# yinwoods/k8s-scheduler

Hardware: AMD Instinct MI355X
Metric: pod-node evaluations/sec (higher is better)
Workload: dtype f64

## Files before the change

### k8s-scheduler_amd/csrc/ksched_commit.h

```cpp
#pragma once

#include <hip/hip_runtime.h>

#include <type_traits>

#ifndef KSCHED_XCHG_DEBUG
#define KSCHED_XCHG_DEBUG 0
#endif

#include "ksched_pipe.h"

namespace ksched {

namespace {

constexpr int kSpcHashBits = 11;
constexpr int kSpcHash = 1 << kSpcHashBits;
template <bool LAG3>
constexpr int spc_slots() { return LAG3 ? 192 : 128; }
static_assert(spc_slots<true>() + 1 <= kRescueMaxT, "RescueReq::ti must hold the persistent commit's touched slots");
constexpr int kSpcInvalid = kSpcHash - 1;
constexpr int kGS = 14;

constexpr uint64_t kSkipKeyBits = 0x7ff8000000000badull;
__device__ __forceinline__ double skip_key() { return __longlong_as_double((long long)kSkipKeyBits); }
__device__ __forceinline__ float screen_y(int64_t a, double y) {
    return (a > 0 && a < (1ll << 52)) ? (float)y : __builtin_nanf("");
}

struct alignas(16) TouchY {
    float c, m, p, w;
};
__device__ __forceinline__ TouchY touch_stage(int64_t a0, int64_t a1, int64_t a2, double y0, double y1, double y2) {
    return TouchY{screen_y(a0, y0), screen_y(a1, y1), screen_y(a2, y2), 0.0f};
}
__device__ __forceinline__ bool touch_need(float qc, float qm, float qp, float thr, const TouchY &ty, int64_t rc, int64_t rm,
                                           int64_t rp, int64_t n0, int64_t n1, int64_t n2, bool active, float *v) {
    bool lo;
    *v = screen_pair(qc, qm, qp, ty.c, ty.m, ty.p, n0 >= rc, n1 >= rm, n2 >= rp, &lo);
    return active && !(*v < thr);
// ... 47 lines not shown
    int32_t *gs;
    double *pbk;
    int64_t *pbx;
    int32_t *ctl;
    int32_t *own;
    uint64_t *GS;
    float *thr;
    int16_t *x2s;
    float *rb2;
};

__device__ __forceinline__ uint32_t spc_hash(int32_t idx) {
    return ((uint32_t)idx * 2654435761u) >> (32 - kSpcHashBits);
}

__device__ __forceinline__ int spc_pos_insert(int32_t *hk, int32_t idx, bool *existed = nullptr) {
    uint32_t h = spc_hash(idx);
    for (;;) {
        if (h != kSpcInvalid) {
            const int32_t prev = atomicCAS(&hk[h], -1, idx);
            if (prev == -1 || prev == idx) {
                if (existed) *existed = prev == idx;
                return (int)h;
            }
        }
        h = (h + 1) & (kSpcHash - 1);
    }
}

__device__ __forceinline__ int64_t rl64(int64_t v, int src) {
    const uint32_t hi = (uint32_t)__builtin_amdgcn_readlane((int)((uint64_t)v >> 32), src);
    const uint32_t lo = (uint32_t)__builtin_amdgcn_readlane((int)(uint32_t)(uint64_t)v, src);
    return (int64_t)(((uint64_t)hi << 32) | lo);
}

__device__ __forceinline__ void persist_plan(const CommitArgs &A, bool truncated, int64_t cursor) {
    PersistLocal *L = A.loc;
    const int64_t n1 = L->plan[(A.batch + kPipeLag - 1) % kPlanRing];
    int64_t nx = truncated ? cursor : (n1 < 0 ? -1 : n1 + A.B);
    if (nx >= A.pods.p) nx = -1;
    L->plan[(A.batch + kPipeLag) % kPlanRing] = nx;
    st_coh(A.plan2, (uint64_t)nx);
}

__device__ __forceinline__ void stage_state(double *o, const int64_t *a) {
    for (int r = 0; r < 3; ++r) {
        const double f = (double)a[r];
        o[r] = f;
        o[3 + r] = recip_or_zero(a[r], f);
    }
}

__device__ __forceinline__ void lds_order() {
    __builtin_amdgcn_fence(__ATOMIC_RELEASE, "wavefront");
    __builtin_amdgcn_wave_barrier();
    __builtin_amdgcn_fence(__ATOMIC_ACQUIRE, "wavefront");
}

template <int PRIO, int DOM, bool LAB, bool F53>
__device__ __forceinline__ double lane_key(bool f, int64_t rc, int64_t rm, int64_t rp, double rcf, double rmf,
                                           double rpf, int64_t n0, int64_t n1, int64_t n2, double y3, float pr) {
    const double nf0 = (double)n0, nf1 = (double)n1, nf2 = (double)n2;
    const double ny0 = recip_or_zero(n0, nf0), ny1 = recip_or_zero(n1, nf1), ny2 = recip_or_zero(n2, nf2);
    double k;
    const bool el = pair_key_fast<PRIO, DOM, F53>(f, rc, rm, rp, rcf, rmf, rpf, n0, n1, n2, nf0, nf1, nf2, ny0, ny1,
                                                  ny2, y3, pr, &k);
// ... 180 lines not shown
            if (wave == 0) {
                if (lane == 0) {
                    L->cursor = ho.cursor;
                    L->plan[(A.batch + kPipeLag - 1) % kPlanRing] = ho.plan_next;
                    L->rseq = ho.rseq;
                    persist_plan(A, false, ho.cursor);
                    st_coh(A.cursor_at, (uint64_t)ho.cursor);
                    drain_stores();
                    put_handoff(A.ctl, A.batch, 0, ho.cursor, ho.rseq, L->plan[(A.batch + kPipeLag) % kPlanRing]);
                }
                publish_committed<COH>(A);
            }
            return 1;
        }
    } else {
        const int64_t cursor = load_i64<COH>(&A.ctl->cursor);
        if (p0 < 0 || p0 >= A.pods.p || p0 != cursor) {
            if (!wait()) return 0;
            if (wave == 0) {
                if (lane == 0) {
                    A.xout->count = 0;
                    if (p0 >= 0 && p0 < A.pods.p) add_i64<COH>(&A.ctl->stats[3], 1);
                    plan_after_commit<COH>(A, false, cursor);
                }
                publish_committed<COH>(A);
            }
            return 1;
        }
    }
    const bool dbg = A.dbg != nullptr;
    uint64_t t_start = dbg ? __builtin_amdgcn_s_memtime() : 0;
    uint64_t t_pre = 0;
    uint64_t t_s1 = 0, t_s2 = 0, t_s3 = 0, t_mark = 0;
    SpcSmem m;
    {
        char *p = smem;
        m.pbk = reinterpret_cast<double *>(p); p += (size_t)kSpcWaves * 64 * sizeof(double);
        m.pbx = reinterpret_cast<int64_t *>(p); p += (size_t)kSpcWaves * 64 * sizeof(int64_t);
        m.LK = reinterpret_cast<double *>(p); p += (size_t)K * 64 * sizeof(double);
        m.GS = reinterpret_cast<uint64_t *>(p); p += 64 * kGS * sizeof(uint64_t);
        m.D = reinterpret_cast<int8_t *>(p); p += 64 * 64;
        m.T = reinterpret_cast<SpcSlot *>(p); p += (size_t)spc_slots<LAG3>() * sizeof(SpcSlot);
        m.LI = reinterpret_cast<int32_t *>(p); p += (size_t)K * 64 * sizeof(int32_t);
        m.HP = reinterpret_cast<int32_t *>(p); p += (size_t)K * 64 * sizeof(int32_t);
        m.hk = reinterpret_cast<int32_t *>(p); p += kSpcHash * sizeof(int32_t);
        m.tkc = reinterpret_cast<uint32_t *>(p); p += 64 * sizeof(uint32_t);
        m.ti = reinterpret_cast<int32_t *>(p); p += spc_slots<LAG3>() * sizeof(int32_t);
        m.fcg = reinterpret_cast<int32_t *>(p); p += 64 * sizeof(int32_t);
        m.dfacc = reinterpret_cast<int32_t *>(p); p += 64 * sizeof(int32_t);
        m.gn = reinterpret_cast<int32_t *>(p); p += 64 * sizeof(int32_t);
        m.gq = reinterpret_cast<int32_t *>(p); p += 64 * sizeof(int32_t);
        m.gs = reinterpret_cast<int32_t *>(p); p += 64 * sizeof(int32_t);
        m.ctl = reinterpret_cast<int32_t *>(p); p += 4 * sizeof(int32_t);
        m.thr = reinterpret_cast<float *>(p); p += 64 * sizeof(float);
        m.x2s = reinterpret_cast<int16_t *>(p); p += 64 * sizeof(int16_t);
        m.S = reinterpret_cast<double *>(p);
        m.own = reinterpret_cast<int32_t *>(m.pbk);
        m.s0 = reinterpret_cast<int64_t *>(m.D);
        m.iy = reinterpret_cast<double *>(m.GS);
        m.iyt = reinterpret_cast<TouchY *>(m.iy + 128 * 6);
        m.rb2 = reinterpret_cast<float *>(m.dfacc);
    }
    const int nb = (int)((A.pods.p - p0 < A.B) ? A.pods.p - p0 : A.B);
    const bool pj = lane < nb;
    const LanePods lp = pre ? *pre : load_lane_pods<LAB>(A.pods, p0, nb);
    const int64_t rc = lp.rc, rm = lp.rm, rp = lp.rp;
// ... 204 lines not shown
            L->rseq = ho.rseq;
        }
        if (p0 != ho.cursor) {
            if (wave == 0) {
                if (lane == 0) {
                    __hip_atomic_fetch_add(reinterpret_cast<unsigned long long *>(&A.ctl->stats[3]), 1ull,
                                           __ATOMIC_RELAXED, __HIP_MEMORY_SCOPE_AGENT);
                    persist_plan(A, false, ho.cursor);
                    st_coh(A.cursor_at, (uint64_t)ho.cursor);
                    drain_stores();
                    put_handoff(A.ctl, A.batch, 0, ho.cursor, ho.rseq, L->plan[(A.batch + kPipeLag) % kPlanRing]);
                }
                publish_committed<COH>(A);
            }
            return 1;
        }
        n1 = ho.n1;
#if KSCHED_XCHG_DEBUG
        if (A.xp && A.xp->xdbg && wave == 0) {
            int64_t x = lane < n1 ? (int64_t)dbg_mix((uint64_t)xi.idx ^ ((uint64_t)xi.cur[0] << 20), (uint64_t)xi.cur[1] ^
                                                     (uint64_t)xi.cur[2] ^ (uint64_t)xi.sb[0], lane) : 0;
            x = wave_sum_i64(x);
            dbg_x1 = (uint64_t)x;
        }
#endif
        if (wave == 0) {
            int h = 0;
            bool dup = false;
            if (lane < n1) {
                h = spc_pos_insert(m.hk, xi.idx);
                dup = (m.tkc[h >> 5] >> (h & 31)) & 1u;
            }
            const uint64_t nm = __ballot(lane < n1 && !dup);
            const int slot = dup ? m.own[h] : n2 + __popcll(nm & ((1ull << lane) - 1ull));
            if (lane < n1) {
                SpcSlot &x = m.T[slot];
                x.idx = xi.idx; x.mine = 0;
                for (int r = 0; r < 3; ++r) { m.s0[lane * 3 + r] = xi.sb[r]; x.sb[r] = xi.cur[r]; x.cur[r] = xi.cur[r]; }
                x.labels = xi.labels; x.price = xi.price; x.pad = 0;
                m.ti[slot] = xi.idx;
                m.gs[lane] = slot;
                if constexpr (SCR) {
                    double st[6];
                    stage_state(st, xi.cur);
#pragma unroll
                    for (int r = 0; r < 6; ++r) m.iy[lane * 6 + r] = st[r];
                    m.iyt[lane] = touch_stage(xi.cur[0], xi.cur[1], xi.cur[2], st[3], st[4], st[5]);
                } else {
                    stage_state(m.iy + lane * 6, xi.cur);
                }
                if (dup) m.x2s[slot] = -1;
                else atomicOr(&m.tkc[h >> 5], 1u << (h & 31));
            }
            if (lane == 0) m.ctl[3] = n2 + __popcll(nm);
        }
        __syncthreads();
        if (tid == 0 && A.trace_row) A.trace_row[23] = wall_clock64();
        nin = m.ctl[3];
        key_inherited(n1, [&](int e) { return (int)m.gs[e]; });
        __syncthreads();
        if (tid == 0 && A.trace_row) A.trace_row[24] = wall_clock64();
    }

    int32_t fcc = 0;
    double rbk = -__builtin_inf();
    int32_t rbi = kNoIdx, rbs = -1;
    constexpr bool RB2 = COH && PRIO == kPrioResource && DOM == kDomAll;
    bool trk = false;
    int cv = 0, cut = 0;
    int32_t my_idx = 0, my_feas = 0;
    int32_t my_src = 0;
    double my_score = 0.0;
    int32_t my_g = -2, my_q = -1, my_s = -1, my_h = kSpcInvalid;
    int nT = nin, done = nb, W = 64;
    int nresc = 0;
    int rcredit = 0, rmax = 0;
    if constexpr (COH) {
        const int c = A.loc->rescue_credit + A.rescue_rate;
        rcredit = c < 4 * A.rescue_cap ? c : 4 * A.rescue_cap;
        rmax = rcredit >= 2 * A.rescue_cap ? A.rescue_max : A.rescue_low;
    }
    int64_t placed = 0, nrounds = 0, nfail = 0, niters = 0, nseq = 0;
    if (wave == 0) {
        int64_t ds2 = 0;
        double xk = -__builtin_inf();
        int32_t xix = kNoIdx, xe = -1;
        if (LAG3 && A.batch >= 2 && n2 > 0 && pj) {
            ds2 = (int64_t)smv[0];
            xk = __longlong_as_double((long long)smv[1]);
            xix = (int32_t)(uint32_t)smv[2];
            xe = (int32_t)(smv[2] >> 32);
        }
        fcc = pj ? (int32_t)(fc0v + m.dfacc[lane] + ds2) : 0;
        cut = cut0;
#pragma unroll
        for (int q = 0; q < K; ++q) cv += m.LI[q * 64 + lane] != kNoIdx;
        for (int w = 0; w < kSpcWaves; ++w) {
            const double k = m.pbk[w * 64 + lane];
            const int64_t x = m.pbx[w * 64 + lane];
            const int32_t xi = (int32_t)(uint32_t)x;
            if (k != -__builtin_inf() && better(k, xi, rbk, rbi)) { rbk = k; rbi = xi; rbs = (int32_t)(x >> 32); }
        }
        if (LAG3 && xix != kNoIdx) {
            if (m.x2s[xe] >= 0) {
                if (better(xk, xix, rbk, rbi)) { rbk = xk; rbi = xix; rbs = m.x2s[xe]; }
            } else {
                for (int e = 0; e < n2; ++e) {
                    if (m.x2s[e] < 0) continue;
                    const double k = Srow[m.x2s[e]];
                    const int32_t xi = m.ti[m.x2s[e]];
                    if (k != -__builtin_inf() && better(k, xi, rbk, rbi)) { rbk = k; rbi = xi; rbs = m.x2s[e]; }
                }
            }
        }
        if (lane == 0) { m.ctl[0] = 0; m.ctl[2] = 0; }
// ... 46 lines not shown
            }
        }
        for (; t < nT; ++t) {
            const double v = Srow[t];
            const int32_t x = m.ti[t];
            const bool u0 = v != -__builtin_inf() && better(v, x, k0, i0);
            if constexpr (T2) { const double o0 = u0 ? k0 : v; q0 = o0 > q0 ? o0 : q0; }
            if (u0) { k0 = v; i0 = x; s0 = t; }
        }
        q0 = q1 > q0 ? q1 : q0;
        if (k1 != -__builtin_inf() && better(k1, i1, k0, i0)) {
            q0 = k0 > q0 ? k0 : q0;
            k0 = k1; i0 = i1; s0 = s1;
        } else {
            q0 = k1 > q0 ? k1 : q0;
        }
        rbk = k0; rbi = i0; rbs = s0;
        if constexpr (T2) m.rb2[lane] = __double2float_ru(q0);
    };
    int c = 0;
    if (COH && tid == 0 && A.trace_row) A.trace_row[25] = wall_clock64();
    uint64_t *const tr1 = (COH && tid == 0) ? A.trace_row : nullptr;
    bool first = true;
    const uint64_t t_pro = dbg ? __builtin_amdgcn_s_memtime() - t_start : 0;
    for (;;) {
        if (dbg) t_mark = __builtin_amdgcn_s_memtime();
        if (wave == 0) {
            const int cend = (c + W < nb) ? c + W : nb;
            lds_order();
            for (int w = lane * 4; w < kSpcHash; w += 256) *reinterpret_cast<int4 *>(m.own + w) = make_int4(64, 64, 64, 64);
            lds_order();
            const uint64_t fitm = __ballot(fcc != 0);
            const bool act = lane >= c && lane < cend && ((fitm >> lane) & 1);
            int32_t hp[K];
            uint32_t am = 0;
#pragma unroll
            for (int qq = 0; qq < K; ++qq) hp[qq] = m.HP[qq * 64 + lane];
#pragma unroll
            for (int qq = 0; qq < K; ++qq) {
                const int pos = hp[qq];
                am |= ((m.tkc[pos >> 5] >> (pos & 31)) & 1u) ? 0u : (1u << qq);
            }
            if (!act) am = 0;
            int32_t pq = -1, ph = kSpcInvalid;
            for (int it = 0;; ++it) {
                ++niters;
                int32_t nq = -1, nh = kSpcInvalid;
                if (am) {
#pragma unroll
                    for (int qq = K - 1; qq >= 0; --qq) {
                        const bool ok = (((am >> qq) & 1u) != 0u) & (m.own[hp[qq]] >= lane);
                        nq = ok ? qq : nq;
                        nh = ok ? hp[qq] : nh;
                    }
                }
                const bool changed = __ballot(act && nq != pq) != 0;
                if (act && pq >= 0) m.own[ph] = 64;
                lds_order();
                pq = nq; ph = nh;
                if (!changed && it > 0) break;
                if (act && pq >= 0) atomicMin(&m.own[ph], lane);
                lds_order();
            }
            const uint64_t gm = __ballot(act && pq >= 0);
            if (lane >= c && lane < cend) {
                my_g = act ? (pq >= 0 ? 0 : -1) : -2;
                my_q = pq;
                my_h = act && pq >= 0 ? ph : kSpcInvalid;
                my_s = act && pq >= 0 ? nT + __popcll(gm & ((1ull << lane) - 1ull)) : -1;
            }
            const bool in = lane >= c && lane < cend;
            if (in && my_g == 0) my_g = m.LI[my_q * 64 + lane];
            m.gn[lane] = in ? my_g : -2;
            m.gq[lane] = my_q;
            m.gs[lane] = my_s;
            m.fcg[lane] = 0;
            if (lane == 0) { m.ctl[0] = c; m.ctl[1] = cend; }
        }
        __syncthreads();
        if (first && tr1) tr1[49] = wall_clock64();
        if (dbg) { const uint64_t t = __builtin_amdgcn_s_memtime(); t_s1 += t - t_mark; t_mark = t; }
        const int rc0 = m.ctl[0], rce = m.ctl[1];
        {
            double pk = -__builtin_inf();
            int32_t pi = kNoIdx, ps = -1;
            if (wave == 0 && lane >= rc0 && lane < rce && m.gn[lane] >= 0) {
                const uint64_t *src = reinterpret_cast<const uint64_t *>(A.lists + (size_t)lane * K + m.gq[lane]) + 2;
                uint64_t v[5];
#pragma unroll
                for (int w = 0; w < 5; ++w) v[w] = COH ? ld_coh(src + w) : src[w];
                const int64_t n0 = wsub((int64_t)v[0], rc), n1 = wsub((int64_t)v[1], rm), n2 = wsub((int64_t)v[2], 1);
                const double nf0 = (double)n0, nf1 = (double)n1, nf2 = (double)n2;
                uint64_t *o = m.GS + (size_t)lane * kGS;
                if constexpr (SCR) {
                    const double ny0 = recip_or_zero(n0, nf0), ny1 = recip_or_zero(n1, nf1), ny2 = recip_or_zero(n2, nf2);
                    SpcSlot &x = m.T[my_s];
                    x.idx = my_g; x.mine = 1;
                    x.sb[0] = (int64_t)v[0]; x.sb[1] = (int64_t)v[1]; x.sb[2] = (int64_t)v[2];
                    x.cur[0] = n0; x.cur[1] = n1; x.cur[2] = n2;
                    x.labels = v[3]; x.price = __uint_as_float((uint32_t)v[4]); x.pad = 0;
                    m.ti[my_s] = my_g;
                    *reinterpret_cast<TouchY *>(o) = touch_stage(n0, n1, n2, ny0, ny1, ny2);
// ... 115 lines not shown
            if (fcj == 0) {
                kind = 0;
            } else if (my_g >= 0) {
                uk = m.LK[my_q * 64 + lane];
                kind = (has_t && better(tk, ti, uk, my_g)) ? 2 : 1;
            } else if (my_g == -2) {
                kind = 4;
            } else if (!cut) {
                kind = has_t ? 2 : 0;
            } else if (cv > 0) {
                const double lk = m.LK[(cv - 1) * 64 + lane];
                const int32_t lx = m.LI[(cv - 1) * 64 + lane];
                kind = (has_t && better(tk, ti, lk, lx)) ? 2 : 3;
            } else {
                kind = 3;
            }
            const bool guessed_commit = my_g >= 0;
            const bool valid = (kind == 0 && !guessed_commit) || (kind == 1);
            const bool inw = lane >= c && lane < cend;
            const uint64_t bad = __ballot(inw && !valid);
            int f = bad ? (int)__builtin_ctzll(bad) : cend;
            const bool conf = lane >= c && lane < f;
            if (conf) {
                my_idx = kind == 1 ? my_g : (fcj == 0 ? -1 : -2);
                my_src = 1 + kind + 8 * my_q;
                my_score = kind == 1 ? (PRIO == kPrioPrice ? 0.0 - uk : uk) : 0.0;
                my_feas = fcj;
                if (guessed_commit) atomicOr(&m.tkc[my_h >> 5], 1u << (my_h & 31));
            }
            placed += __popcll(__ballot(conf && kind == 1));
            const int ncg = __popcll(__ballot(conf && guessed_commit));
            nT += ncg;
            if (f < nb) {
                float b2 = trk ? m.rb2[lane] : 0.0f;
                for (int k = c; k < f; ++k) {
                    const int32_t g = __builtin_amdgcn_readlane(my_g, k);
                    if (g < 0) continue;
                    const int s = __builtin_amdgcn_readlane(my_s, k);
                    const double v = Srow[s];
                    fcc += m.D[k * 64 + lane];
                    const bool up = v != -__builtin_inf() && better(v, g, rbk, rbi);
                    if (trk) {
                        const double o = up ? rbk : v;
                        b2 = o > (double)b2 ? __double2float_ru(o) : b2;
                    }
                    rbk = up ? v : rbk; rbi = up ? g : rbi; rbs = up ? s : rbs;
                }
                if (trk) m.rb2[lane] = b2;
            }
            if (f < cend) {
                ++nfail;
                int kf = __builtin_amdgcn_readlane(kind, f);
                int32_t fcf = __builtin_amdgcn_readlane(fcj, f);
                double wk = readlane_f64(tk, f);
                int32_t wi = __builtin_amdgcn_readlane(ti, f);
                int s = __builtin_amdgcn_readlane(ts, f);
                const int fr = f;
                for (;;) {
                int qf = -1;
                if (kf == 4) {
                    const int cvf = __builtin_amdgcn_readlane(cv, f);
                    bool free_ = false;
                    int32_t e = kNoIdx;
                    if (lane < cvf) {
                        e = m.LI[lane * 64 + f];
                        const int pos = m.HP[lane * 64 + f];
                        free_ = !((m.tkc[pos >> 5] >> (pos & 31)) & 1u);
                    }
                    const uint64_t fm = __ballot(free_);
                    const bool ht = wi != kNoIdx;
                    if (fm) {
                        qf = __builtin_ctzll(fm);
                        const int32_t ue = __builtin_amdgcn_readlane(e, qf);
                        const double ukf = m.LK[qf * 64 + f];
                        if (ht && better(wk, wi, ukf, ue)) kf = 2;
                        else { kf = 1; wk = ukf; wi = ue; }
                    } else if (!__builtin_amdgcn_readlane(cut, f)) {
                        kf = ht ? 2 : 0;
                    } else if (cvf > 0) {
                        const double lk = m.LK[(cvf - 1) * 64 + f];
                        const int32_t lx = m.LI[(cvf - 1) * 64 + f];
                        kf = (ht && better(wk, wi, lk, lx)) ? 2 : 3;
                    } else {
                        kf = 3;
                    }
                }
                kf = __builtin_amdgcn_readfirstlane(kf);
                bool rescued = false;
                RescueOut ro{};
                if constexpr (COH) {
                    bool afford = kf == 3 && A.rescue && nresc < rmax && 4 * (nresc + 1) <= rcredit;
                    if (afford && A.rescue_look) {
                        bool risk = false;
                        if (lane > f && lane < nb && cut) {
                            risk = true;
#pragma unroll
                            for (int q = 0; q < K; ++q) {
                                if (q < cv) {
                                    const int pos = m.HP[q * 64 + lane];
                                    risk = risk && ((m.tkc[pos >> 5] >> (pos & 31)) & 1u);
                                }
                            }
                        }
                        const int n = nresc + 1 + __popcll(__ballot(risk));
                        afford = n <= rmax && 4 * n <= rcredit;
                    }
                    if (afford &&
                        commit_rescue(A, f, rl64(rc, f), rl64(rm, f), rl64(rp, f), (uint64_t)rl64((int64_t)sel, f),
                                      m.ti, nT, &ro)) {
                        ++nresc;
                        if (lane == 0) ++L->stats[4];
#if KSCHED_XCHG_DEBUG
                        if (A.xp && A.xp->xdbg && lane == 0 && nresc <= 4 && A.dbg_act >= 0 && A.dbg_act < A.xp->xdbg_cap) {
                            uint64_t *d = A.xp->xdbg + xdbg_commit_off(A.xp->xdbg_cap, A.xp->B, A.xp->R, K) +
                                          (size_t)A.xp->xdbg_cap * 8 + (size_t)A.dbg_act * 8 + 2 * (nresc - 1);
                            d[0] = (uint64_t)(uint32_t)f | (uint64_t)(uint32_t)ro.idx << 32;
                            d[1] = (uint64_t)__double_as_longlong(ro.key);
                        }
#endif
                        if constexpr (SCR) rekey_row(f, wk, wi, s);
                        const bool ht = wi != kNoIdx;
                        if (ro.idx != kNoIdx && !(ht && better(wk, wi, ro.key, ro.idx))) {
                            kf = 1;
                            rescued = true;
                            wk = ro.key;
                            wi = ro.idx;
                        } else {
                            kf = ht ? 2 : 0;
                        }
                    }
                }
                if (kf == 3) {
                    done = f;
                } else {
                    if (lane == f) {
                        my_idx = kf == 0 ? (fcf == 0 ? -1 : -2) : wi;
                        my_src = 1000 + kf + (rescued ? 10 : 0) + 100 * (qf + 1) + 10000 * (int)(nseq & 63);
                        my_score = kf == 0 ? 0.0 : (PRIO == kPrioPrice ? 0.0 - wk : wk);
                        my_feas = fcf;
                    }
                    if (kf != 0) {
                        ++placed;
                        int64_t b0, b1, b2;
                        uint64_t lab;
                        float pr;
                        if (kf == 1 && rescued) {
                            b0 = ro.a[0]; b1 = ro.a[1]; b2 = ro.a[2]; lab = ro.labels; pr = ro.price;
                            s = nT++;
                        } else if (kf == 1) {
                            int64_t ra[3];
                            load_rec_state<COH>(A.lists + (size_t)f * K + qf, ra, &lab, &pr);
                            b0 = ra[0]; b1 = ra[1]; b2 = ra[2];
                            s = nT++;
                        } else {
                            const SpcSlot &x = m.T[s];
                            b0 = x.cur[0]; b1 = x.cur[1]; b2 = x.cur[2]; lab = x.labels; pr = x.price;
                        }
                        const int64_t n0 = wsub(b0, rl64(rc, f)), n1 = wsub(b1, rl64(rm, f)), n2 = wsub(b2, 1);
                        const bool fo = fits(rc, rm, rp, sel, b0, b1, b2, lab, LAB);
                        const bool fn = fits(rc, rm, rp, sel, n0, n1, n2, lab, LAB);
                        fcc += (int32_t)fn - (int32_t)fo;
                        double kv;
                        if constexpr (SCR) {
                            const int64_t nn[3] = {n0, n1, n2};
                            double st[6];
                            stage_state(st, nn);
                            const bool any = touch_column<PRIO, DOM, F53>(
                                screen_req(rc), screen_req(rm), screen_req(rp), m.thr[lane],
                                touch_stage(n0, n1, n2, st[3], st[4], st[5]), lane > f && pj, fn, rc, rm, rp, rcf, rmf, rpf,
                                n0, n1, n2, st, y3, pr, &kv);
                            if (A.dbg && lane == 0) {
                                atomicAdd(reinterpret_cast<unsigned long long *>(&A.dbg[20]), 1ull);
                                if (any) atomicAdd(reinterpret_cast<unsigned long long *>(&A.dbg[21]), 1ull);
                            }
                        } else {
                            kv = lane_key<PRIO, DOM, LAB, F53>(fn, rc, rm, rp, rcf, rmf, rpf, n0, n1, n2, y3, pr);
                        }
                        Srow[s] = kv;
                        if (lane == 0) {
                            SpcSlot &x = m.T[s];
                            if (kf == 1) {
                                x.idx = wi;
                                x.sb[0] = b0; x.sb[1] = b1; x.sb[2] = b2;
                                x.labels = lab; x.price = pr; x.pad = 0;
                                m.ti[s] = wi;
                                const int pos = rescued ? spc_pos_insert(m.hk, wi) : m.HP[qf * 64 + f];
                                m.tkc[pos >> 5] |= 1u << (pos & 31);
                            }
                            x.mine = 1;
                            x.cur[0] = n0; x.cur[1] = n1; x.cur[2] = n2;
                        }
                        lds_order();
                        const bool up = kv != -__builtin_inf() && better(kv, wi, rbk, rbi);
                        const bool hold = rbs == s;
                        const bool worse = !up && hold;
                        bool keep = false;
                        if (trk) {
                            const float b2 = m.rb2[lane];
                            keep = worse && kv > (double)b2;
                            const double o = up ? rbk : kv;
                            if (!hold && o > (double)b2) m.rb2[lane] = __double2float_ru(o);
                        }
                        const bool rescan = worse && !keep;
                        rbk = (up || keep) ? kv : rbk; rbi = up ? wi : rbi; rbs = up ? s : rbs;
                        const bool anyr = __ballot(rescan) != 0;
                        const bool anyw = RB2 && __ballot(worse) != 0;
                        if (RB2 && A.dbg && lane == 0 && anyw) {
                            atomicAdd(reinterpret_cast<unsigned long long *>(&A.dbg[23]), 1ull);
                            if (!anyr) atomicAdd(reinterpret_cast<unsigned long long *>(&A.dbg[24]), 1ull);
                        }
                        if (anyr) {
                            const uint64_t tr0 = RB2 && dbg ? __builtin_amdgcn_s_memtime() : 0;
                            const bool trk_was = trk;
                            if (trk) {
                                if (rescan) rescan_row(std::true_type{});
                            } else {
                                if (rescan) rescan_row(std::false_type{});
                                if constexpr (RB2) {
                                    trk = __ballot(rescan && rbs == s) != 0;
                                    if (trk) m.rb2[lane] = __builtin_inff();
                                }
                            }
                            if (RB2 && dbg) {
                                const uint64_t dt = __builtin_amdgcn_s_memtime() - tr0;
                                if (lane == 0) {
                                    const int o = trk_was ? 27 : 25;
                                    atomicAdd(reinterpret_cast<unsigned long long *>(&A.dbg[o]), 1ull);
                                    atomicAdd(reinterpret_cast<unsigned long long *>(&A.dbg[o + 1]), (unsigned long long)dt);
                                    if (A.trace_row) A.trace_row[29] += dt;
                                }
                            }
                        }
                    }
                }
                if (kf != 2 || f + 1 >= nb) break;
                ++f;
                ++nseq;
                fcf = __builtin_amdgcn_readlane(fcc, f);
                kf = fcf == 0 ? 0 : 4;
// ... 22 lines not shown

    auto store_out = [&]() {
        const bool bad_out = COH && lane < done && (my_idx < -2 || my_idx >= (1 << 30));
        const uint64_t bm = __ballot(bad_out);
        if (bm) {
            const int l = (int)__builtin_ctzll(bm);
            const int src = __builtin_amdgcn_readlane(my_src, l);
            const int val = __builtin_amdgcn_readlane(my_idx, l);
            if (lane == 0 && atomicCAS(A.err, 0, kErrBadIndex) == 0 && A.xp && A.xp->prog) {
                A.xp->prog[kProgWords * (A.xp->G + A.xp->B) + 3] =
                    (uint64_t)A.batch << 40 | (uint64_t)l << 32 | (uint64_t)(uint32_t)src;
                A.xp->prog[kProgWords * (A.xp->G + A.xp->B) + 4] = (uint64_t)(uint32_t)val;
            }
        }
        if (lane < done) {
            A.out.idx[p0 + lane] = my_idx;
            A.out.score[p0 + lane] = my_score;
            A.out.feas[p0 + lane] = my_feas;
        }
    };
    if (!COH) store_out();
    int base = 0;
    for (int t0 = 0; t0 < nT; t0 += 64) {
        const int t = t0 + lane;
        const bool mine = t < nT && m.T[t].mine;
        const uint64_t mask = __ballot(mine);
        if (mine) {
            const SpcSlot &x = m.T[t];
            XRec o;
            o.idx = x.idx; o.pad = 0;
            o.sb[0] = x.sb[0]; o.sb[1] = x.sb[1]; o.sb[2] = x.sb[2];
            o.cur[0] = x.cur[0]; o.cur[1] = x.cur[1]; o.cur[2] = x.cur[2];
            o.labels = x.labels; o.price = x.price; o.pad2 = 0;
            const int slot = base + __popcll(mask & ((1ull << lane) - 1));
            store_xrec<COH>(A.xout->e, slot, o, (uint32_t)(A.batch + 1));
        }
        base += __popcll(mask);
    }
#if KSCHED_XCHG_DEBUG
    if (COH && A.xp && A.xp->xdbg && A.dbg_act >= 0 && A.dbg_act < A.xp->xdbg_cap) {
        int64_t x = lane < done ? (int64_t)dbg_mix((uint64_t)(uint32_t)my_idx, (uint64_t)__double_as_longlong(my_score), lane) : 0;
        x = wave_sum_i64(x);
        if (lane == 0) A.xp->xdbg[xdbg_commit_off(A.xp->xdbg_cap, A.xp->B, A.xp->R, K) + (size_t)A.dbg_act * 8 + 3] = (uint64_t)x;
    }
#endif
    if (lane == 0) {
        if (COH) {
            st_coh(&A.xout->count, (uint64_t)(uint32_t)base | (uint64_t)(uint32_t)A.batch << 32);
            L->cursor = p0 + done;
            persist_plan(A, done < nb, p0 + done);
            st_coh(A.cursor_at, (uint64_t)L->cursor);
            drain_stores();
            if (A.xp) jitter_at(A.xp->jitter, A.batch, 101);
            put_handoff(A.ctl, A.batch, base, L->cursor, L->rseq, L->plan[(A.batch + kPipeLag) % kPlanRing]);
            if (A.trace_row) A.trace_row[53] = wall_clock64();
        } else {
            A.xout->count = base;
            store_i64<COH>(&A.ctl->cursor, p0 + done);
            add_i64<COH>(&A.ctl->stats[0], 1);
            add_i64<COH>(&A.ctl->stats[1], (done < nb) ? 1 : 0);
            add_i64<COH>(&A.ctl->stats[2], placed);
            plan_after_commit<COH>(A, done < nb, p0 + done);
        }
#if KSCHED_XCHG_DEBUG
        if (COH && A.xp && A.xp->xdbg && A.dbg_act >= 0 && A.dbg_act < A.xp->xdbg_cap) {
            uint64_t *d = A.xp->xdbg + xdbg_commit_off(A.xp->xdbg_cap, A.xp->B, A.xp->R, K) + (size_t)A.dbg_act * 8;
            d[0] = (uint64_t)p0;
            d[1] = (uint64_t)done | (uint64_t)nresc << 16 | (uint64_t)nrounds << 32 | (uint64_t)nfail << 48;
            d[2] = (uint64_t)n1 | (uint64_t)n2 << 16 | (uint64_t)nin << 32 | (uint64_t)base << 48;
            d[4] = dbg_x1;
            d[7] = (uint64_t)A.batch;
        }
#endif
        if (A.trace_row)
            A.trace_row[16] = (uint64_t)nrounds | (uint64_t)nresc << 16 | (uint64_t)done << 24 | (uint64_t)nfail << 32 |
                              (uint64_t)nseq << 48;
        if (A.dbg) {
            A.dbg[12] += nrounds; A.dbg[13] += nfail; A.dbg[14] += 1; A.dbg[5] += niters;
            A.dbg[0] += t_pro; A.dbg[1] += t_s1; A.dbg[2] += t_s2; A.dbg[3] += t_s3;
            if (A.trace_row) { A.trace_row[18] = t_pro; A.trace_row[19] = t_s1; A.trace_row[20] = t_s2; A.trace_row[21] = t_s3; }
            A.dbg[4] += __builtin_amdgcn_s_memtime() - t_start;
            A.dbg[6] += t_pre;
        }
    }
    if (COH && A.xp) jitter_at(A.xp->jitter, A.batch, 102);
    publish_committed<COH>(A);
    if (COH) {
        store_out();
        if (lane == 0) {
            unsigned long long *st = reinterpret_cast<unsigned long long *>(A.ctl->stats);
            __hip_atomic_fetch_max(reinterpret_cast<unsigned long long *>(&A.ctl->cursor), (unsigned long long)L->cursor,
                                   __ATOMIC_RELAXED, __HIP_MEMORY_SCOPE_AGENT);
            __hip_atomic_fetch_add(st + 0, 1ull, __ATOMIC_RELAXED, __HIP_MEMORY_SCOPE_AGENT);
            if (done < nb) __hip_atomic_fetch_add(st + 1, 1ull, __ATOMIC_RELAXED, __HIP_MEMORY_SCOPE_AGENT);
            __hip_atomic_fetch_add(st + 2, (unsigned long long)placed, __ATOMIC_RELAXED, __HIP_MEMORY_SCOPE_AGENT);
            if (nresc) __hip_atomic_fetch_add(st + 4, (unsigned long long)nresc, __ATOMIC_RELAXED, __HIP_MEMORY_SCOPE_AGENT);
        }
        if (threadIdx.x == 0) A.loc->rescue_credit = rcredit - 4 * nresc;
    }
    return 1;
}

template <int K, int NT = kSpcThreads, bool LAG3 = false>
constexpr size_t spc_small_bytes() {
    return (size_t)(NT / 64) * 64 * 16 + (size_t)K * 64 * 8 + 64 * kGS * 8 + 64 * 64 + spc_slots<LAG3>() * sizeof(SpcSlot) +
           (size_t)K * 64 * 8 + (size_t)kSpcHash * 4 + 64 * 4 + spc_slots<LAG3>() * 4 + 5 * 64 * 4 + 16 + 64 * 4 + 64 * 2;
}
template <int K, int NT = kSpcThreads, bool LAG3 = false>
constexpr size_t spc_lds_bytes() {
    return (size_t)64 * (spc_slots<LAG3>() + 1) * 8 + (size_t)(NT / 64) * 64 * 16 + (size_t)K * 64 * 12 +
           spc_slots<LAG3>() * sizeof(SpcSlot) + (size_t)kSpcHash * 4 + (size_t)K * 64 * 4 + 64 * 4 +
           spc_slots<LAG3>() * 4 + 5 * 64 * 4 + 16 + 64 * kGS * 8 + 64 * 4 + 64 * 2 + 64 * 64;
}
// ... 10 lines not shown
```

### k8s-scheduler_amd/csrc/ksched_diag.hip

```cpp
#include <cstdio>
#include <cstdlib>
#include <cstring>

#include "ksched_ctx.h"

namespace ksched {

static int env_int(const char *name, int dflt) {
    const char *v = std::getenv(name);
    return v && *v ? std::atoi(v) : dflt;
}
static std::string env_str(const char *name) {
    const char *v = std::getenv(name);
    return v ? v : "";
}

void read_env(ksched_diag *d) {
    d->trace = env_int("KSCHED_PERSIST_TRACE", 0) != 0;
    d->trace_dump = env_str("KSCHED_TRACE_DUMP");
    d->trace_wg = env_str("KSCHED_TRACE_WG");
    d->xchg_dump = env_str("KSCHED_XCHG_DUMP");
    d->commit_stamps = env_int("KSCHED_COMMIT_STAMPS", 0) != 0;
    d->merge_stamps = env_int("KSCHED_MERGE_STAMPS", 0) != 0;
    d->debug = env_int("KSCHED_DEBUG", 0) != 0;
// ... 52 lines not shown
        sum[4] += (double)(int64_t)(at(b, 4) - at(b, 3));
        sum[5] += (double)(int64_t)(at(b, 3) - at(b - 1, 4));
        sum[6] += (double)(int64_t)(at(b, 6) - at(b - L, 4));
        sum[7] += (double)(int64_t)(at(b, 0) - at(b, 6));
        sum[8] += (double)(int64_t)(at(b, 5) - at(b, 0));
        sum[9] += (double)(int64_t)(at(b, 7) - at(b, 1));
        sum[10] += (double)(int64_t)(at(b, 8) - at(b, 0));
        sum[11] += (double)(int64_t)(at(b, 9) - at(b, 8));
        sum[12] += (double)(int64_t)(at(b, 10) - at(b, 9));
        sum[13] += (double)(int64_t)(at(b, 5) - at(b, 10));
        sum[14] += (double)(int64_t)(at(b, 15) - at(b - 1, 4));
        sum[15] += (double)(int64_t)(at(b, 3) - at(b, 15));
        if (at(b, 11) && at(b, 12)) {
            ++nscr;
            scr[0] += (double)(int64_t)(at(b, 11) - at(b, 0));
            const uint64_t bar = at(b, 37) ? at(b, 37) : at(b, 11);
            scr[5] += (double)(int64_t)(bar - at(b, 11));
            scr[1] += (double)(int64_t)(at(b, 12) - bar);
            scr[2] += (double)(int64_t)(at(b, 14) - at(b, 12));
            scr[3] += (double)(int64_t)(at(b, 8) - at(b, 14));
            scr[4] += (double)(uint32_t)at(b, 13);
            const uint32_t pairs = (uint32_t)(at(b, 13) >> 32);
            if (pairs != 0xffffffffu) { ++npair; pairs_sum += pairs; }
        }
    }
    if (c->d->dbg) {
        int64_t hd[32];
        if (hipMemcpy(hd, c->d->dbg, sizeof(hd), hipMemcpyDeviceToHost) == hipSuccess && hd[14] && hd[16])
            fprintf(stderr, "persist commit screen: export(b-1) entries %lld keyed exactly %.4f | guessed columns %lld, "
                    "exactly %.4f | sequential columns %lld, exactly %.4f | rescue re-keys %lld\n", (long long)hd[16],
                    (double)hd[17] / std::max<int64_t>(1, hd[16]), (long long)hd[18], (double)hd[19] / std::max<int64_t>(1, hd[18]),
                    (long long)hd[20], (double)hd[21] / std::max<int64_t>(1, hd[20]), (long long)hd[22]);
        if (hd[14])
            fprintf(stderr, "persist commit: batches=%lld rounds/batch %.3f guess iterations/round %.2f failures %lld | "
                    "cycles/batch: before the wait %.0f (other waves %.0f) entry to past the wait %.0f (poll %.0f, poll + barrier %.0f, early read sufficed %.3f, early inh read sufficed %lld of %lld) | prologue %.0f guess %.0f evaluate %.0f check %.0f total %.0f\n",
                    (long long)hd[14], (double)hd[12] / hd[14], (double)hd[5] / std::max<int64_t>(1, hd[12]),
                    (long long)hd[13], (double)hd[6] / hd[14], (double)hd[9] / hd[14] / 11.0, (double)hd[7] / hd[14], (double)hd[10] / hd[14], (double)hd[11] / hd[14], (double)hd[15] / hd[14], (long long)hd[29], (long long)hd[30], (double)hd[0] / hd[14],
                    (double)hd[1] / hd[14], (double)hd[2] / hd[14], (double)hd[3] / hd[14], (double)hd[4] / hd[14]);
        if (hd[14])
            fprintf(stderr, "persist commit rescans: steps with a worsened holder %lld, every holder kept %lld | plain rescans "
                    "%lld, %.0f cycles each | with the second-best key %lld, %.0f cycles each\n", (long long)hd[23],
                    (long long)hd[24], (long long)hd[25], (double)hd[26] / std::max<int64_t>(1, hd[25]), (long long)hd[27],
                    (double)hd[28] / std::max<int64_t>(1, hd[27]));
    }
    if (c->d->mdbg) {
        int64_t hm[8];
        if (hipMemcpy(hm, c->d->mdbg, sizeof(hm), hipMemcpyDeviceToHost) == hipSuccess && hm[7]) {
            const double nwg = (double)hm[7];
            fprintf(stderr, "persist merge: merges=%lld | cycles/merge: loads %.0f rank-heads %.0f barrier %.0f "
                    "global-heads %.0f rank-entries %.0f write %.0f\n", (long long)hm[7], hm[0] / nwg, hm[1] / nwg,
                    hm[2] / nwg, hm[3] / nwg, hm[4] / nwg, hm[5] / nwg);
        }
    }
    if (!cnt) return;
    const double us = 0.01 / (double)cnt;
    fprintf(stderr,
            "persist trace: %lld batches, period %.2f us | to-score %.2f score %.2f merge %.2f to-commit %.2f "
            "commit %.2f commit-gap %.2f (to loop top %.2f, top to past the wait %.2f) | wg0: poll %.2f apply %.2f "
            "score %.2f (rows %.2f slowest-wave %.2f fold %.2f stores %.2f) | merger poll %.2f\n",
            (long long)cnt, 0.01 * (double)(int64_t)(at(last, 4) - at(first, 4)) / (double)std::max<int64_t>(1, last - first),
            sum[0] * us, sum[1] * us, sum[2] * us, sum[3] * us, sum[4] * us, sum[5] * us, sum[14] * us, sum[15] * us, sum[6] * us, sum[7] * us,
            sum[8] * us, sum[10] * us, sum[11] * us, sum[12] * us, sum[13] * us, sum[9] * us);
    if (nscr)
        fprintf(stderr, "persist screen (WG 0 wave 0): %lld of %lld batches screened | pass 1 / seed pass %.2f us, other waves "
                "%.2f us, bound %.2f us, pass 2 / single pass %.2f us, exact phase %.2f us (%.2f of the workgroup's %d rows needed; pair lists in %lld batches, "
                "%.1f pairs each)\n", (long long)nscr, (long long)cnt,
// ... 189 lines not shown
```

### k8s-scheduler_amd/ksched/engine.py

```python
from __future__ import annotations

import ctypes as C
from typing import Optional

import numpy as np

from . import _lib as L

PIPELINES = {0: "none", 1: "exact", 2: "stream", 3: "stream-sequential", 4: "persistent"}


def _i64(a):
    return np.ascontiguousarray(a, dtype=np.int64)


class Group:

    def __init__(self, nranks: int, device: int = -1):
        h = C.c_void_p()
        L.check(L.lib().ksched_group_create(int(nranks), int(device), C.byref(h)), what="group_create")
        self._h = h
        self.nranks = nranks

    def close(self):
# ... 192 lines not shown
                                             L.ptr(rp, C.c_int64), L.ptr(sel, C.c_uint64)), "upload_pods")
        self.p = p

    def run(self):
        self._chk(L.lib().ksched_run(self._ctx), "run")

    def sync(self):
        self._chk(L.lib().ksched_sync(self._ctx), "sync")

    def results(self):
        oi = np.empty(self.p, np.int32); os_ = np.empty(self.p, np.float64); of = np.empty(self.p, np.int32)
        self._chk(L.lib().ksched_download_results(self._ctx, self.p, L.ptr(oi, C.c_int32), L.ptr(os_, C.c_double),
                                                  L.ptr(of, C.c_int32)), "download_results")
        return oi, os_, of

    def stats(self) -> dict:
        s = L.Stats()
        self._chk(L.lib().ksched_get_stats(self._ctx, C.byref(s)), "get_stats")
        return dict(pods=s.pods, placed=s.placed, batches=s.batches, truncations=s.truncations,
                    pair_evals=s.pair_evals, device_ms=s.device_ms, kernel_ms=list(s.kernel_ms),
                    kernel_launches=list(s.kernel_launches), kernel_pairs=list(s.kernel_pairs),
                    pipeline=PIPELINES.get(int(s.pipeline), str(int(s.pipeline))), rescues=s.rescues,
                    exact_rows=s.exact_rows, scan_rows=s.scan_rows)

    def seed_stats(self) -> dict:
        w = (C.c_int64 * 5)()
        self._chk(L.lib().ksched_get_seed_stats(self._ctx, w), "get_seed_stats")
        return dict(seeded_scans=w[0], seed_rows=w[1], zero_bound_scans=w[2], after_unscreened=w[3], past_cap=w[4])

    def commit_stamps(self) -> dict:
        w = (C.c_int64 * 32)()
        self._chk(L.lib().ksched_get_commit_stamps(self._ctx, 32, w), "get_commit_stamps")
        return dict(rounds=w[12], failed_guesses=w[13], batches=w[14], early_merged=w[15], early_inh=w[29],
                    early_inh_tried=w[30])

    def set_timing(self, on: bool, every: int = 0):
        self._chk(L.lib().ksched_set_timing(self._ctx, int(bool(on)), int(every)), "set_timing")

    def set_timeout(self, ms: int):
        self._chk(L.lib().ksched_set_timeout(self._ctx, int(ms)), "set_timeout")

    def schedule(self, req_cpu, req_mem, req_pods, selector=None):
        self.upload_pods(req_cpu, req_mem, req_pods, selector)
        self.run()
        self.sync()
        return self.results()

    def _schedule_with(self, name, req_cpu, req_mem, req_pods, selector, extra, tail=()):
        rc, rm, rp = _i64(req_cpu), _i64(req_mem), _i64(req_pods)
        p = rc.shape[0]
        assert rm.shape[0] == p and rp.shape[0] == p
        sel = None if selector is None else np.ascontiguousarray(selector, dtype=np.uint64)
        ext_args = extra(p)
        oi = np.empty(p, np.int32); os_ = np.empty(p, np.float64); of = np.empty(p, np.int32)
        self._chk(getattr(L.lib(), "ksched_" + name)(self._ctx, p, L.ptr(rc, C.c_int64), L.ptr(rm, C.c_int64),
                                                     L.ptr(rp, C.c_int64), L.ptr(sel, C.c_uint64), *ext_args,
                                                     L.ptr(oi, C.c_int32), L.ptr(os_, C.c_double), L.ptr(of, C.c_int32),
                                                     *tail), name)
        self.p = p
        return oi, os_, of

    def schedule_gangs(self, req_cpu, req_mem, req_pods, selector, gang_off, gang_min=None):
        off = _i64(gang_off)
        ng = off.shape[0] - 1
        gmin = None if gang_min is None else np.ascontiguousarray(gang_min, dtype=np.int32)
        assert ng >= 0 and (gmin is None or gmin.shape[0] == ng)
        gp = np.empty(ng, np.int32)
# ... 171 lines not shown
```

Measured before the change: 301.5 billion.

## Speed up commit guess loop with two-entry fast path and batched LDS gathers

Rewrites the persistent commit's guess iteration so each lane first checks only its two lowest candidate entries, read with paired inline-asm LDS loads. It falls back to a full K-entry scan, done with batched LDS gathers, only when some lane needs a third candidate. Prefix lane counts now use mbcnt instead of popcount on a mask, and debug counters and split timers are added for full scans and sequential resolution. The aim is to cut per-iteration LDS latency and register pressure in the hot guess loop. The cost is extra inline assembly with explicit waitcnt stalls and a divergent fallback path.

```diff
diff --git a/k8s-scheduler_amd/csrc/ksched_commit.h b/k8s-scheduler_amd/csrc/ksched_commit.h
--- a/k8s-scheduler_amd/csrc/ksched_commit.h
+++ b/k8s-scheduler_amd/csrc/ksched_commit.h
@@ -6,6 +6,9 @@
 
 #ifndef KSCHED_XCHG_DEBUG
 #define KSCHED_XCHG_DEBUG 0
+#endif
+#ifndef KSCHED_COMMIT_SPLIT
+#define KSCHED_COMMIT_SPLIT 0
 #endif
 
 #include "ksched_pipe.h"
@@ -119,6 +122,70 @@
     const uint32_t hi = (uint32_t)__builtin_amdgcn_readlane((int)((uint64_t)v >> 32), src);
     const uint32_t lo = (uint32_t)__builtin_amdgcn_readlane((int)(uint32_t)(uint64_t)v, src);
     return (int64_t)(((uint64_t)hi << 32) | lo);
+}
+
+__device__ __forceinline__ int lanes_below(uint64_t mask) {
+    return (int)__builtin_amdgcn_mbcnt_hi((uint32_t)(mask >> 32), __builtin_amdgcn_mbcnt_lo((uint32_t)mask, 0u));
+}
+
+__device__ __forceinline__ uint32_t lds_addr(const void *p) {
+    return (uint32_t)(uintptr_t)(__attribute__((address_space(3))) const void *)p;
+}
+
+__device__ __forceinline__ void lds_read2(uint32_t a0, uint32_t a1, int32_t &o0, int32_t &o1) {
+#if defined(__HIP_DEVICE_COMPILE__)
+    asm volatile("ds_read_b32 %0, %2\n\tds_read_b32 %1, %3\n\ts_waitcnt lgkmcnt(0)"
+                 : "=&v"(o0), "=&v"(o1) : "v"(a0), "v"(a1) : "memory");
+#else
+    o0 = o1 = 0; (void)a0; (void)a1;
+#endif
+}
+
+template <int N, int SHIFT>
+__device__ __forceinline__ void lds_gather(uint32_t hp_at, uint32_t base2, int32_t (&hp)[N], int32_t (&w)[N]) {
+    static_assert(N == 4 || N == 8, "lds_gather: 4 or 8 entries");
+#if defined(__HIP_DEVICE_COMPILE__)
+    if constexpr (N == 4) {
+        asm volatile("ds_read_b32 %0, %8\n\tds_read_b32 %1, %8 offset:256\n\t"
+                     "ds_read_b32 %2, %8 offset:512\n\tds_read_b32 %3, %8 offset:768\n\t"
+                     "s_waitcnt lgkmcnt(0)\n\t"
+                     "v_lshrrev_b32 %4, %10, %0\n\tv_lshrrev_b32 %5, %10, %1\n\t"
+                     "v_lshrrev_b32 %6, %10, %2\n\tv_lshrrev_b32 %7, %10, %3\n\t"
+                     "v_lshl_add_u32 %4, %4, 2, %9\n\tv_lshl_add_u32 %5, %5, 2, %9\n\t"
+                     "v_lshl_add_u32 %6, %6, 2, %9\n\tv_lshl_add_u32 %7, %7, 2, %9\n\t"
+                     "ds_read_b32 %4, %4\n\tds_read_b32 %5, %5\n\tds_read_b32 %6, %6\n\tds_read_b32 %7, %7\n\t"
+                     "s_waitcnt lgkmcnt(0)"
+                     : "=&v"(hp[0]), "=&v"(hp[1]), "=&v"(hp[2]), "=&v"(hp[3]), "=&v"(w[0]), "=&v"(w[1]), "=&v"(w[2]),
+                       "=&v"(w[3])
+                     : "v"(hp_at), "v"(base2), "i"(SHIFT)
+                     : "memory");
+    } else {
+        asm volatile("ds_read_b32 %0, %16\n\tds_read_b32 %1, %16 offset:256\n\t"
+                     "ds_read_b32 %2, %16 offset:512\n\tds_read_b32 %3, %16 offset:768\n\t"
+                     "ds_read_b32 %4, %16 offset:1024\n\tds_read_b32 %5, %16 offset:1280\n\t"
+                     "ds_read_b32 %6, %16 offset:1536\n\tds_read_b32 %7, %16 offset:1792\n\t"
+                     "s_waitcnt lgkmcnt(0)\n\t"
+                     "v_lshrrev_b32 %8, %18, %0\n\tv_lshrrev_b32 %9, %18, %1\n\t"
+                     "v_lshrrev_b32 %10, %18, %2\n\tv_lshrrev_b32 %11, %18, %3\n\t"
+                     "v_lshrrev_b32 %12, %18, %4\n\tv_lshrrev_b32 %13, %18, %5\n\t"
+                     "v_lshrrev_b32 %14, %18, %6\n\tv_lshrrev_b32 %15, %18, %7\n\t"
+                     "v_lshl_add_u32 %8, %8, 2, %17\n\tv_lshl_add_u32 %9, %9, 2, %17\n\t"
+                     "v_lshl_add_u32 %10, %10, 2, %17\n\tv_lshl_add_u32 %11, %11, 2, %17\n\t"
+                     "v_lshl_add_u32 %12, %12, 2, %17\n\tv_lshl_add_u32 %13, %13, 2, %17\n\t"
+                     "v_lshl_add_u32 %14, %14, 2, %17\n\tv_lshl_add_u32 %15, %15, 2, %17\n\t"
+                     "ds_read_b32 %8, %8\n\tds_read_b32 %9, %9\n\tds_read_b32 %10, %10\n\tds_read_b32 %11, %11\n\t"
+                     "ds_read_b32 %12, %12\n\tds_read_b32 %13, %13\n\tds_read_b32 %14, %14\n\tds_read_b32 %15, %15\n\t"
+                     "s_waitcnt lgkmcnt(0)"
+                     : "=&v"(hp[0]), "=&v"(hp[1]), "=&v"(hp[2]), "=&v"(hp[3]), "=&v"(hp[4]), "=&v"(hp[5]), "=&v"(hp[6]),
+                       "=&v"(hp[7]), "=&v"(w[0]), "=&v"(w[1]), "=&v"(w[2]), "=&v"(w[3]), "=&v"(w[4]), "=&v"(w[5]),
+                       "=&v"(w[6]), "=&v"(w[7])
+                     : "v"(hp_at), "v"(base2), "i"(SHIFT)
+                     : "memory");
+    }
+#else
+    for (int u = 0; u < N; ++u) hp[u] = w[u] = 0;
+    (void)hp_at; (void)base2;
+#endif
 }
 
 __device__ __forceinline__ void persist_plan(const CommitArgs &A, bool truncated, int64_t cursor) {
@@ -365,6 +432,8 @@
     uint64_t t_start = dbg ? __builtin_amdgcn_s_memtime() : 0;
     uint64_t t_pre = 0;
     uint64_t t_s1 = 0, t_s2 = 0, t_s3 = 0, t_mark = 0;
+    const bool sdbg = KSCHED_COMMIT_SPLIT && dbg;
+    uint64_t t_fold = 0, t_probe = 0, t_pod = 0, t_load = 0;
     SpcSmem m;
     {
         char *p = smem;
@@ -635,7 +704,7 @@
                 dup = (m.tkc[h >> 5] >> (h & 31)) & 1u;
             }
             const uint64_t nm = __ballot(lane < n1 && !dup);
-            const int slot = dup ? m.own[h] : n2 + __popcll(nm & ((1ull << lane) - 1ull));
+            const int slot = dup ? m.own[h] : n2 + lanes_below(nm);
             if (lane < n1) {
                 SpcSlot &x = m.T[slot];
                 x.idx = xi.idx; x.mine = 0;
@@ -684,6 +753,7 @@
         rmax = rcredit >= 2 * A.rescue_cap ? A.rescue_max : A.rescue_low;
     }
     int64_t placed = 0, nrounds = 0, nfail = 0, niters = 0, nseq = 0;
+    int nfull = 0;
     if (wave == 0) {
         int64_t ds2 = 0;
         double xk = -__builtin_inf();
@@ -796,26 +866,45 @@
             lds_order();
             const uint64_t fitm = __ballot(fcc != 0);
             const bool act = lane >= c && lane < cend && ((fitm >> lane) & 1);
-            int32_t hp[K];
+            constexpr int G = K < 8 ? K : 8;
+            const uint32_t hp_at = lds_addr(m.HP + lane), own_at = lds_addr(m.own);
             uint32_t am = 0;
 #pragma unroll
-            for (int qq = 0; qq < K; ++qq) hp[qq] = m.HP[qq * 64 + lane];
-#pragma unroll
-            for (int qq = 0; qq < K; ++qq) {
-                const int pos = hp[qq];
-                am |= ((m.tkc[pos >> 5] >> (pos & 31)) & 1u) ? 0u : (1u << qq);
+            for (int g = 0; g < K; g += G) {
+                int32_t hp[G], tw[G];
+                lds_gather<G, 5>(hp_at + g * 256, lds_addr(m.tkc), hp, tw);
+#pragma unroll
+                for (int u = 0; u < G; ++u) am |= (((uint32_t)tw[u] >> (hp[u] & 31)) & 1u) ? 0u : (1u << (g + u));
             }
             if (!act) am = 0;
+            const uint32_t am1 = am & (am - 1u), amr = am1 & (am1 - 1u);
+            const int32_t q0 = am ? (int32_t)__builtin_ctz(am) : 0, q1 = am1 ? (int32_t)__builtin_ctz(am1) : 0;
+            int32_t h0, h1;
+            lds_read2(hp_at + q0 * 256, hp_at + q1 * 256, h0, h1);
             int32_t pq = -1, ph = kSpcInvalid;
             for (int it = 0;; ++it) {
                 ++niters;
-                int32_t nq = -1, nh = kSpcInvalid;
-                if (am) {
-#pragma unroll
-                    for (int qq = K - 1; qq >= 0; --qq) {
-                        const bool ok = (((am >> qq) & 1u) != 0u) & (m.own[hp[qq]] >= lane);
-                        nq = ok ? qq : nq;
-                        nh = ok ? hp[qq] : nh;
+                int32_t nq, nh;
+                {
+                    int32_t o0, o1;
+                    lds_read2(own_at + h0 * 4, own_at + h1 * 4, o0, o1);
+                    const bool ok0 = am != 0u && o0 >= lane, ok1 = am1 != 0u && o1 >= lane;
+                    nq = ok0 ? q0 : (ok1 ? q1 : -1);
+                    nh = ok0 ? h0 : (ok1 ? h1 : kSpcInvalid);
+                    if (__ballot(amr != 0u && !ok0 && !ok1) != 0) {
+                        ++nfull;
+                        nq = -1; nh = kSpcInvalid;
+#pragma unroll
+                        for (int g = K - G; g >= 0; g -= G) {
+                            int32_t hp[G], ow[G];
+                            lds_gather<G, 0>(hp_at + g * 256, own_at, hp, ow);
+#pragma unroll
+                            for (int u = G - 1; u >= 0; --u) {
+                                const bool ok = (((am >> (g + u)) & 1u) != 0u) & (ow[u] >= lane);
+                                nq = ok ? g + u : nq;
+                                nh = ok ? hp[u] : nh;
+                            }
+                        }
                     }
                 }
                 const bool changed = __ballot(act && nq != pq) != 0;
@@ -831,7 +920,7 @@
                 my_g = act ? (pq >= 0 ? 0 : -1) : -2;
                 my_q = pq;
                 my_h = act && pq >= 0 ? ph : kSpcInvalid;
-                my_s = act && pq >= 0 ? nT + __popcll(gm & ((1ull << lane) - 1ull)) : -1;
+                my_s = act && pq >= 0 ? nT + lanes_below(gm) : -1;
             }
             const bool in = lane >= c && lane < cend;
             if (in && my_g == 0) my_g = m.LI[my_q * 64 + lane];
@@ -1013,6 +1102,7 @@
             const int ncg = __popcll(__ballot(conf && guessed_commit));
             nT += ncg;
             if (f < nb) {
+                const uint64_t tf0 = sdbg ? __builtin_amdgcn_s_memtime() : 0;
                 float b2 = trk ? m.rb2[lane] : 0.0f;
                 for (int k = c; k < f; ++k) {
                     const int32_t g = __builtin_amdgcn_readlane(my_g, k);
@@ -1028,6 +1118,7 @@
                     rbk = up ? v : rbk; rbi = up ? g : rbi; rbs = up ? s : rbs;
                 }
                 if (trk) m.rb2[lane] = b2;
+                if (sdbg) t_fold += __builtin_amdgcn_s_memtime() - tf0;
             }
             if (f < cend) {
                 ++nfail;
@@ -1039,6 +1130,7 @@
                 const int fr = f;
                 for (;;) {
                 int qf = -1;
+                const uint64_t tp0 = sdbg ? __builtin_amdgcn_s_memtime() : 0;
                 if (kf == 4) {
                     const int cvf = __builtin_amdgcn_readlane(cv, f);
                     bool free_ = false;
@@ -1067,6 +1159,7 @@
                     }
                 }
                 kf = __builtin_amdgcn_readfirstlane(kf);
+                if (sdbg) t_probe += __builtin_amdgcn_s_memtime() - tp0;
                 bool rescued = false;
                 RescueOut ro{};
                 if constexpr (COH) {
@@ -1122,6 +1215,7 @@
                     }
                     if (kf != 0) {
                         ++placed;
+                        const uint64_t tc0 = sdbg ? __builtin_amdgcn_s_memtime() : 0;
                         int64_t b0, b1, b2;
                         uint64_t lab;
                         float pr;
@@ -1133,6 +1227,10 @@
                             load_rec_state<COH>(A.lists + (size_t)f * K + qf, ra, &lab, &pr);
                             b0 = ra[0]; b1 = ra[1]; b2 = ra[2];
                             s = nT++;
+                            if (sdbg) {
+                                asm volatile("s_waitcnt vmcnt(0)" ::: "memory");
+                                t_load += __builtin_amdgcn_s_memtime() - tc0;
+                            }
                         } else {
                             const SpcSlot &x = m.T[s];
                             b0 = x.cur[0]; b1 = x.cur[1]; b2 = x.cur[2]; lab = x.labels; pr = x.price;
@@ -1186,6 +1284,7 @@
                         rbk = (up || keep) ? kv : rbk; rbi = up ? wi : rbi; rbs = up ? s : rbs;
                         const bool anyr = __ballot(rescan) != 0;
                         const bool anyw = RB2 && __ballot(worse) != 0;
+                        if (sdbg) t_pod += __builtin_amdgcn_s_memtime() - tc0;
                         if (RB2 && A.dbg && lane == 0 && anyw) {
                             atomicAdd(reinterpret_cast<unsigned long long *>(&A.dbg[23]), 1ull);
                             if (!anyr) atomicAdd(reinterpret_cast<unsigned long long *>(&A.dbg[24]), 1ull);
@@ -1274,7 +1373,7 @@
             o.sb[0] = x.sb[0]; o.sb[1] = x.sb[1]; o.sb[2] = x.sb[2];
             o.cur[0] = x.cur[0]; o.cur[1] = x.cur[1]; o.cur[2] = x.cur[2];
             o.labels = x.labels; o.price = x.price; o.pad2 = 0;
-            const int slot = base + __popcll(mask & ((1ull << lane) - 1));
+            const int slot = base + lanes_below(mask);
             store_xrec<COH>(A.xout->e, slot, o, (uint32_t)(A.batch + 1));
         }
         base += __popcll(mask);
@@ -1319,8 +1418,12 @@
                               (uint64_t)nseq << 48;
         if (A.dbg) {
             A.dbg[12] += nrounds; A.dbg[13] += nfail; A.dbg[14] += 1; A.dbg[5] += niters;
+            A.dbg[8] += nfull; A.dbg[31] += nseq;
             A.dbg[0] += t_pro; A.dbg[1] += t_s1; A.dbg[2] += t_s2; A.dbg[3] += t_s3;
             if (A.trace_row) { A.trace_row[18] = t_pro; A.trace_row[19] = t_s1; A.trace_row[20] = t_s2; A.trace_row[21] = t_s3; }
+            if (KSCHED_COMMIT_SPLIT && A.trace_row) {
+                A.trace_row[33] = t_fold; A.trace_row[34] = t_probe; A.trace_row[35] = t_pod; A.trace_row[36] = t_load;
+            }
             A.dbg[4] += __builtin_amdgcn_s_memtime() - t_start;
             A.dbg[6] += t_pre;
         }
diff --git a/k8s-scheduler_amd/csrc/ksched_diag.hip b/k8s-scheduler_amd/csrc/ksched_diag.hip
--- a/k8s-scheduler_amd/csrc/ksched_diag.hip
+++ b/k8s-scheduler_amd/csrc/ksched_diag.hip
@@ -108,6 +108,9 @@
                     (double)hd[17] / std::max<int64_t>(1, hd[16]), (long long)hd[18], (double)hd[19] / std::max<int64_t>(1, hd[18]),
                     (long long)hd[20], (double)hd[21] / std::max<int64_t>(1, hd[20]), (long long)hd[22]);
         if (hd[14])
+            fprintf(stderr, "persist commit guess: iterations %lld, of them past the two lowest entries (all K scanned) %lld | "
+                    "pods resolved one by one %lld\n", (long long)hd[5], (long long)hd[8], (long long)hd[31]);
+        if (hd[14])
             fprintf(stderr, "persist commit: batches=%lld rounds/batch %.3f guess iterations/round %.2f failures %lld | "
                     "cycles/batch: before the wait %.0f (other waves %.0f) entry to past the wait %.0f (poll %.0f, poll + barrier %.0f, early read sufficed %.3f, early inh read sufficed %lld of %lld) | prologue %.0f guess %.0f evaluate %.0f check %.0f total %.0f\n",
                     (long long)hd[14], (double)hd[12] / hd[14], (double)hd[5] / std::max<int64_t>(1, hd[12]),
diff --git a/k8s-scheduler_amd/ksched/engine.py b/k8s-scheduler_amd/ksched/engine.py
--- a/k8s-scheduler_amd/ksched/engine.py
+++ b/k8s-scheduler_amd/ksched/engine.py
@@ -248,7 +248,7 @@
         w = (C.c_int64 * 32)()
         self._chk(L.lib().ksched_get_commit_stamps(self._ctx, 32, w), "get_commit_stamps")
         return dict(rounds=w[12], failed_guesses=w[13], batches=w[14], early_merged=w[15], early_inh=w[29],
-                    early_inh_tried=w[30])
+                    early_inh_tried=w[30], guess_iterations=w[5], full_scans=w[8], one_by_one=w[31])
 
     def set_timing(self, on: bool, every: int = 0):
         self._chk(L.lib().ksched_set_timing(self._ctx, int(bool(on)), int(every)), "set_timing")
```

Measured after the change: 307.3 billion (median of 6 runs). +2.0%, better.
